# shenwei356/kmcp

Measured on AMD Instinct MI355X. Metric: reads/sec searched (150bp, k=21) vs GTDB-scale index, higher is better.
Workload: dtype u32 bitwise (bit-sliced counters), u64 hashes; 1 GPU; gtdb-scale synthetic: 32 blocks x 14976 cols x 968700 sigs (58.03 GB), 150bp k=21; batch_reads=524288, read_len=150, k=21, num_hashes=1, index_bytes=58029004800, index_bytes_this_rank=58029004800, blocks=32, columns=479232, parallelism=block-shard x1, search_flags=-t 0.55 -c 10 -m 30 -f 0.01 -u 256 -s qcov

## Files before the change

kmcp_amd/csrc/common.hpp:

```cpp
#pragma once
#include <stdint.h>

#include "../../include/kmcp_gpu.h"

namespace kmcpg {

struct BlockDev {
  const uint8_t* rows;
  uint64_t num_sigs;
  uint64_t magic_hi;
  uint32_t stride;
  uint32_t row_bytes;
  uint32_t ncols;
  uint32_t col_base;
  uint32_t seg0, nsegs;
};

struct Seg {
  uint32_t byte_start, byte_end;
  uint32_t col_base;
  uint32_t ncols;
};

struct ExcRun {
  uint64_t pos;
  uint32_t len;
  uint32_t byte;
};

struct Slot {
  uint32_t block;
  uint32_t tile;
};
constexpr uint32_t SLOT_TILE_BITS = 24, SLOT_MAX_TILES = 255;

struct K1Args {
  const uint8_t* seqs;
  const uint64_t* offs;
  const uint8_t* seqs2;
  const uint64_t* offs2;
  uint32_t n_reads;
  int32_t k;
  int32_t min_qlen;
  int32_t scaled;
  uint64_t max_hash;
  int32_t mode;
  uint32_t w_or_s;
  uint64_t* hashes;
  uint64_t* scratch;
  uint64_t* scratch2;
  int32_t* nk_raw;
  int32_t* nk1;
  int32_t* qlen;
  int32_t* seg_cnt;
  uint32_t segs_max;
  int32_t* nk_adj;
  int32_t dedup_threshold;
  int32_t flags;
  uint32_t* seg_list;
  uint32_t* seg_nflag;
  int32_t seg_only_flagged;
  const uint8_t* codes;
  const ExcRun* exc;
  uint32_t n_exc;
  uint8_t* seqs_w;
  uint32_t* seg_exc;
  const uint64_t* src;
};


struct PackedSrc {
  const uint8_t* codes = nullptr;
  const ExcRun* exc = nullptr;
  uint32_t n_exc = 0;
  uint8_t* text = nullptr;
  uint64_t n_bases = 0;
};
constexpr int K1_WIN_CHUNK = 1024;
struct WindowSrc {
  const uint64_t* src = nullptr;
  const uint64_t* soffs = nullptr;
  const uint64_t* wpre = nullptr;
  const uint64_t* cpre = nullptr;
  uint32_t ns = 0;
  uint64_t n_chunks = 0, sb = 0, step = 0, window = 0;
};

struct DedupArgs {
  const uint64_t* offs;
  const uint64_t* offs2;
  uint32_t n_reads;
  int32_t dedup_threshold;
  int32_t min_matched;
  int32_t lo, hi;
  int32_t n_lo, n_hi;
  int32_t pre;
  int32_t pre_done;
  int32_t key_shift;
  uint64_t* hashes;
  uint64_t* scratch;
  const int32_t* nk_raw;
  int32_t* nk_search;
  uint32_t* fallbacks;
};

constexpr int K2_GATHER_SLOTS = 256;

struct K2Args {
  const BlockDev* blocks;
  const Seg* segs;
  const Slot* slots;
  uint32_t nslots;
  uint32_t n_reads;
  const uint64_t* hashes;
  const uint64_t* offs;
  const uint64_t* offs2;
  const int32_t* nk;
  double min_qcov;
  int32_t min_matched;
  int32_t num_hashes;
  int32_t nt_loads;
  int32_t prune;
  int32_t group_rows;
  int32_t prune_every;
  int32_t split_min;
  int32_t slot_major;
  int32_t tail_sectors;
  int32_t tail_min;
  const uint32_t* long_list;
  uint32_t n_long;
  uint32_t split_chk;
  uint32_t split_chunks;
  uint32_t* long_counts;
  uint32_t ncols_total;
  uint64_t unit_base;
  kmcpg_hit* hits;
  uint64_t hit_cap;
  unsigned long long* counter;
  unsigned long long* gathered;
  const uint16_t* cmin_fpr;
  int32_t cmin_fpr_n;
  int32_t k2_flags;
};
static_assert(sizeof(K2Args) == 208, "k2_flags sits in the tail padding: the argument block of every K2 form keeps its layout");

constexpr int K3_WAVE_CAP = 512, K3_WG_CAP = 4096;
struct K3Args {
  const kmcpg_hit* hits;
  const unsigned long long* n_hits;
  uint64_t hit_cap;
  const int32_t* nk;
  uint32_t n_reads;
  uint32_t n_cols;
  const uint64_t* col_size;
  double min_tcov;
  int32_t sort_mode;
  uint32_t* cnt;
  uint64_t* offs;
  uint64_t* sums;
  kmcpg_pair* pairs;
  uint32_t* bad;
};

constexpr int K3_SET_STATS = 4;
struct K3SetArgs {
  uint32_t n_members;
  uint32_t base[16];
  uint32_t* stats;
};

constexpr uint8_t K4_DROP = 0, K4_KEEP = 1, K4_HOST = 2;
constexpr int K4_STATS = 6;
struct K4Args {
  const kmcpg_pair* pairs;
  const uint64_t* offs;
  uint64_t pair_cap;
  const int32_t* nk;
  uint32_t n_reads;
  uint32_t n_cols;
  int32_t final_n;
  const uint32_t* target_class;
  const uint32_t* species_class;
  uint32_t* cnt;
  uint64_t* sums;
  uint8_t* verdict;
  kmcpg_pair* out_pairs;
  uint64_t* out_offs;
  uint64_t out_cap;
  uint32_t* stats;
};

}
```

kmcp_amd/csrc/engine.hpp:

```cpp
#pragma once
#include <stdlib.h>
#include <hip/hip_runtime.h>
#include <stdint.h>

#include <atomic>
#include <condition_variable>
#include <functional>
#include <memory>
#include <mutex>
#include <string>
#include <vector>

#include "../../include/kmcp_gpu.h"
#include "common.hpp"
#include "dbformat.hpp"
#include "k1_plan.hpp"
#include "fpr.hpp"

int kmcpg_fail(int code, const char* fmt, ...);
std::string& kmcpg_err_ref();

#define HIPCHK(expr)                                                                               \
  do {                                                                                             \
    hipError_t e_ = (expr);                                                                        \
    if (e_ != hipSuccess) return kmcpg_fail(KMCPG_EDEVICE, "%s: %s (%s:%d)", #expr, hipGetErrorString(e_), __FILE__, __LINE__); \
  } while (0)

#define KMCPG_NO_FILES_ONLY(db)                                                                                   \
  do {                                                                                                            \
    if ((db)->files_only) return kmcpg_fail(KMCPG_EUNSUPPORTED, "handle of kmcpg_open_files: index inspection only, open the database directory with kmcpg_open to search it"); \
  } while (0)

#define KMCPG_USE_DEVICE(db)                                                                                      \
  do {                                                                                                            \
    if ((db)->opts.device < 0) return kmcpg_fail(KMCPG_EDEVICE, "metadata-only handle (device -1): no GPU work possible"); \
    HIPCHK(hipSetDevice((db)->opts.device));                                                                      \
  } while (0)

namespace kmcpg {

struct BlockMeta {
  std::string path;
  UnikiHeader h;
  uint32_t col_base = 0;
  bool local = false;
  int local_idx = -1;
  uint32_t stride = 0;
  uint8_t* d_rows = nullptr;
  int group = -1;
  uint32_t byte_off = 0;
};

struct Group {
  uint8_t* d_rows = nullptr;
  uint64_t num_sigs = 0;
  uint32_t stride = 0, row_bytes = 0;
  std::vector<int> members;
};

struct SlotClass {
  int lpr = 0;
  std::vector<Slot> slots;
  Slot* d_slots = nullptr;
  std::vector<Slot> bslots;
  Slot* d_bslots = nullptr;
};

template <typename T>
struct DevBuf {
  T* p = nullptr;
  size_t cap = 0;
  int ensure(size_t n) {
    if (n <= cap) return 0;
    if (p) (void)hipFree(p);
    p = nullptr;
    cap = 0;
    size_t want = n + n / 8 + 64;
    if (hipMalloc((void**)&p, want * sizeof(T)) != hipSuccess) return -1;
    cap = want;
    return 0;
  }
  void release() {
    if (p) (void)hipFree(p);
    p = nullptr;
    cap = 0;
  }
};

}

namespace kmcpg {
struct Exchange;
struct FprBoundTable {
  uint64_t key = 0;
  int n = 0;
  uint16_t* d = nullptr;
  uint16_t* h = nullptr;
};
void release_fpr_bounds(kmcpg_db* db);
int plan_passes(kmcpg_db* front, int device, uint64_t* largest_shard_bytes, uint64_t* free_bytes, uint64_t* reserve_bytes = nullptr);
int open_like(const kmcpg_db* src, const kmcpg_opts* opts, kmcpg_db** out);
struct AsyncState;
void async_release(kmcpg_db* db);
int async_in_flight(kmcpg_db* db);
}

struct kmcpg_db {
  kmcpg_opts opts{};
  kmcpg_info info{};
  std::vector<kmcpg::BlockMeta> blocks;
  std::vector<int> local;
  std::vector<kmcpg::BlockDev> h_blockdev;
  kmcpg::BlockDev* d_blockdev = nullptr;
  std::vector<kmcpg::Group> groups;
  std::vector<kmcpg::BlockDev> h_groupdev;
  kmcpg::BlockDev* d_groupdev = nullptr;
  std::vector<kmcpg::Seg> h_segs;
  kmcpg::Seg* d_segs = nullptr;
  std::vector<kmcpg::SlotClass> classes;
  std::vector<uint32_t> col_block;
  struct ColMeta {
    uint64_t size;
    uint64_t gsize;
    uint32_t tidx;
    uint32_t pad;
  };
  std::vector<ColMeta> col_meta;
  std::unique_ptr<kmcpg::QueryFpr> fpr;
  std::mutex mu;
  std::vector<int> ks_desc;
  kmcpg::AsyncState* async = nullptr;
  struct Workspace {
    kmcpg::DevBuf<uint64_t> w_hashes, w_scratch;
    kmcpg::DevBuf<int32_t> w_nk_raw, w_nk1, w_seg_cnt;
    kmcpg::DevBuf<uint32_t> w_long_list, w_long_meta, w_long_counts;
    kmcpg::DevBuf<uint64_t> w_huge_info;
    kmcpg::DevBuf<uint8_t> w_huge_temp;
    kmcpg::DevBuf<uint32_t> w_dedup_fb;
    kmcpg::DevBuf<uint64_t> w_gathered;
    kmcpg::DevBuf<uint64_t> w_win_h, w_win_kept, w_win_cbase;
    kmcpg::DevBuf<uint32_t> w_win_rank, w_win_cnt;
    hipEvent_t ev = nullptr;
    bool ev_valid = false;
    hipEvent_t in_ev = nullptr, k1_ev = nullptr;
    void release() {
      w_hashes.release(); w_scratch.release(); w_nk_raw.release(); w_nk1.release(); w_seg_cnt.release(); w_long_list.release();
      w_long_meta.release(); w_long_counts.release(); w_huge_info.release(); w_huge_temp.release(); w_gathered.release(); w_dedup_fb.release();
      w_win_h.release(); w_win_kept.release(); w_win_cbase.release(); w_win_rank.release(); w_win_cnt.release();
      if (ev) (void)hipEventDestroy(ev);
      if (in_ev) (void)hipEventDestroy(in_ev);
      if (k1_ev) (void)hipEventDestroy(k1_ev);
      ev = in_ev = k1_ev = nullptr;
      ev_valid = false;
    }
  };
  Workspace ws[2];
  uint64_t ws_calls = 0;
  uint64_t k1_codes_direct = 0, k1_codes_expanded = 0;
  int ws_last = 0;
  hipStream_t k1_stream = nullptr;
  hipEvent_t cobs_ev = nullptr;
  bool cobs_ev_valid = false;
  hipEvent_t fin_ev = nullptr;
  bool fin_ev_valid = false;
  bool synthetic = false;
  bool files_only = false;
  float last_density_ms = -1;
  kmcpg_density_launch last_density{};
  std::vector<kmcpg_db*> shards;
  kmcpg::Exchange* exchange = nullptr;
  std::string exchange_why;
  std::string db_dir;
  int paged_passes = 0, paged_device = 0, paged_rank = -1;
  kmcpg_db* paged_resident = nullptr;
  std::mutex paged_mu;
  uint64_t paged_uploads = 0;
  uint64_t paged_reserve = 0;
  int profiling = 0;
  std::vector<kmcpg_k2_launch> k2_log;
  std::vector<kmcpg_k1_launch> k1_log;
  const uint32_t* k1_left = nullptr;
  std::vector<kmcpg_dedup_launch> dedup_log;
  const uint32_t* dedup_fb = nullptr;
  uint64_t* d_col_size = nullptr;
  kmcpg::DevBuf<uint32_t> w_fin_cnt;
  kmcpg::DevBuf<uint64_t> w_fin_sums;
  std::vector<std::string> set_dirs;
  std::vector<uint32_t> set_col_base;
  bool is_set() const { return set_col_base.size() > 1; }
  uint32_t* d_set_stats = nullptr;
  mutable std::atomic<uint64_t> set_host_segments{0}, set_host_mixed{0};
  uint32_t* d_spec_target = nullptr;
  uint32_t* d_spec_species = nullptr;
  std::vector<uint32_t> h_spec_target, h_spec_species;
  bool spec_on() const { return !h_spec_target.empty(); }
  kmcpg::DevBuf<uint32_t> w_spec_cnt;
  kmcpg::DevBuf<uint64_t> w_spec_sums;
  uint64_t* d_spec_stats = nullptr;
  bool spec_ran = false;
  hipEvent_t spec_ev[2] = {};
  bool spec_timed = false;
  std::vector<kmcpg_k4_launch> k4_log;
  std::vector<kmcpg::FprBoundTable> fpr_bounds;
  hipEvent_t ev[16] = {};
  uint64_t ev_calls = 0;
};


namespace kmcpg {

inline int set_refuse_params(const kmcpg_db* db, const kmcpg_params& p) {
  if (!db->is_set()) return 0;
  const char* what = p.try_se ? "try_se" : (p.do_not_sort ? "do_not_sort" : (p.top_n_scores != 0 ? "top_n_scores != 0" : (p.k != 0 ? "params->k != 0" : nullptr)));
  if (!what) return 0;
  return kmcpg_fail(KMCPG_EUNSUPPORTED, "database set (%zu members): %s is not supported — it acts per member in separate searches and would act per query here; "
                    "search the databases one by one and merge the results with kmcp-merge", db->set_col_base.size(), what);
}
inline int set_refuse_entry(const kmcpg_db* db, const char* entry) {
  if (!db->is_set()) return 0;
  return kmcpg_fail(KMCPG_EUNSUPPORTED, "database set (%zu members): %s is not supported on a set handle", db->set_col_base.size(), entry);
}

inline int specific_refuse_params(const kmcpg_db* db, const kmcpg_params& p) {
  if (!db->spec_on()) return 0;
  const char* what = p.try_se ? "try_se" : (p.top_n_scores != 0 ? "top_n_scores != 0" : (p.k == 0 && db->ks_desc.size() > 1 ? "a database with several k-mer sizes searched with params->k == 0" : nullptr));
  if (!what) return 0;
  return kmcpg_fail(KMCPG_EUNSUPPORTED, "species-specific queries (kmcpg_set_specific): %s is not supported — switch the stage off, or filter the results with kmcp-filter", what);
}
inline int specific_refuse_entry(const kmcpg_db* db, const char* entry) {
  if (!db->spec_on()) return 0;
  return kmcpg_fail(KMCPG_EUNSUPPORTED, "species-specific queries (kmcpg_set_specific): %s is not supported while the stage is on", entry);
}

inline kmcpg_params default_params() {
  kmcpg_params p{};
  p.min_qlen = 30;
  p.min_matched = 10;
  p.min_qcov = 0.55;
  p.min_tcov = 0;
  p.max_fpr = 0.01;
  p.dedup_threshold = 256;
  return p;
}

template <class T>
struct NoInitAlloc : std::allocator<T> {
  template <class U>
  struct rebind {
    using other = NoInitAlloc<U>;
  };
  template <class U, class... A>
  void construct(U* q, A&&... a) {
    if constexpr (sizeof...(A) == 0) ::new ((void*)q) U;
    else ::new ((void*)q) U(std::forward<A>(a)...);
  }
};
template <class T>
struct LineAlloc : NoInitAlloc<T> {
  template <class U>
  struct rebind {
    using other = LineAlloc<U>;
  };
  T* allocate(size_t n) {
    void* q = nullptr;
    if (posix_memalign(&q, 64, std::max<size_t>(64, n * sizeof(T))) != 0) throw std::bad_alloc();
    return (T*)q;
  }
  void deallocate(T* q, size_t) { free(q); }
};
typedef std::vector<kmcpg_match, LineAlloc<kmcpg_match>> MatchVec;

struct ResultOwner {
  std::vector<int32_t> qlen, qkmers, ksize;
  std::vector<uint64_t> offs;
  MatchVec matches;
  std::vector<kmcpg_pair, NoInitAlloc<kmcpg_pair>> pairs;
  bool pairs_mode = false;
};
ResultOwner* result_owner_take();
void result_owner_give(ResultOwner* o);
void result_owner_shape(ResultOwner* o, uint32_t n_reads, bool as_pairs);
int finalize_grouped_into(const kmcpg_db* db, const kmcpg_pair* pairs, const uint64_t* read_offs, const int32_t* qkmers, const int32_t* qlen, uint32_t n_reads,
                          const kmcpg_params& p, ResultOwner* o, uint32_t read_base, uint64_t match_base, uint64_t* kept_out, bool trusted = false,
                          int32_t bound_n = 0, const uint8_t* verdicts = nullptr);
int finalize_grouped_trusted(const kmcpg_db* db, const kmcpg_pair* pairs, const uint64_t* read_offs, const int32_t* qkmers, const int32_t* qlen, uint32_t n_reads,
                             const kmcpg_params& p, kmcpg_result* out, int32_t bound_n, bool as_pairs, const uint8_t* verdicts = nullptr);
void specific_filter_result(const kmcpg_db* db, kmcpg_result* out);
inline int k1_mode(const kmcpg_info& I) { return I.syncmer ? 2 : (I.minimizer ? 1 : 0); }
bool whole_genome_batch(const kmcpg_db* db, uint32_t max_read_len, bool paired);
inline bool fpr_bound_enabled() {
  const char* e = getenv("KMCPG_FPR_BOUND");
  return !(e && atoi(e) == 0);
}
constexpr int kFprBoundAlways = 512;
void result_publish(ResultOwner* o, uint32_t n_reads, int k_used, kmcpg_result* out);
struct DeviceBatch {
  const uint8_t* d_seqs = nullptr;
  const uint64_t* d_offs = nullptr;
  const uint8_t* d_seqs2 = nullptr;
  const uint64_t* d_offs2 = nullptr;
// ... 44 lines not shown
```

kmcp_amd/csrc/k2_cobs.hip:

```cpp
#include <hip/hip_runtime.h>

#include <algorithm>
#include <type_traits>

#include "common.hpp"
#include "csa.hpp"
#include "device_utils.hpp"
#include "kernels.hpp"

namespace kmcpg {

typedef uint32_t u32x4 __attribute__((ext_vector_type(4)));
__device__ __forceinline__ uint4 load_row16(const uint8_t* p, int nt) {
  const u32x4* q = reinterpret_cast<const u32x4*>(p);
  const u32x4 v = nt ? __builtin_nontemporal_load(q) : *q;
  return make_uint4(v.x, v.y, v.z, v.w);
}

typedef const u32x4 __attribute__((address_space(1))) * global_row_ptr;
__device__ __forceinline__ uint4 load_row16_global(const uint8_t* p, int nt) {
  global_row_ptr q = (global_row_ptr)(uintptr_t)p;
  const u32x4 v = nt ? __builtin_nontemporal_load(q) : *q;
  return make_uint4(v.x, v.y, v.z, v.w);
}

__device__ __forceinline__ bool group_col(const Seg* __restrict__ segs, const BlockDev* __restrict__ bd, uint32_t byte, uint32_t bit, uint32_t* col) {
  const Seg* s = segs + bd->seg0;
  for (uint32_t i = 0; i < bd->nsegs; i++, s++) {
    if (byte < s->byte_end) {
      const uint32_t c = (byte - s->byte_start) * 8u + (7u - bit);
      *col = s->col_base + c;
      return byte >= s->byte_start && c < s->ncols;
    }
  }
  return false;
}


struct alignas(16) UnitConst {
  uint64_t ns, mh;
  uint64_t koff;
  uint32_t s16;
  int32_t n;
};

template <int NPL>
__device__ __forceinline__ void k2_emit_tile(const K2Args& a, const BlockDev* __restrict__ bd, uint32_t r, uint32_t boff, uint32_t cmin, bool live,
                                             const uint32_t (&pl)[4][NPL], int lane) {
  const bool emit = live && (cmin >> NPL) == 0;
  uint32_t ge[4];
  uint32_t mine = 0;
#pragma unroll
  for (int d = 0; d < 4; d++) {
    uint32_t v = emit ? 0xffffffffu : 0u;
#pragma unroll
    for (int p = 0; p < NPL; p++) v = ((cmin >> p) & 1u) ? (v & pl[d][p]) : (v | pl[d][p]);
    ge[d] = v;
    mine += (uint32_t)__popc(v);
  }
  if (__ballot(mine != 0) == 0) return;
  uint32_t incl = mine;
#pragma unroll
  for (int off = 1; off < 64; off <<= 1) {
    const uint32_t t = __shfl_up(incl, off);
    if (lane >= off) incl += t;
  }
  const uint32_t total = __shfl(incl, 63);
  unsigned long long base_idx = 0;
  if (lane == 63) base_idx = atomicAdd(a.counter, (unsigned long long)total);
  base_idx = __shfl(base_idx, 63);
  unsigned long long idx = base_idx + (incl - mine);
  uint32_t sg_lo = 1, sg_hi = 0, sg_col = 0;
  const Seg* __restrict__ segs = a.segs + bd->seg0;
  const uint32_t nsegs = bd->nsegs;
#pragma unroll
  for (int d = 0; d < 4; d++) {
    uint32_t w = ge[d];
    while (w) {
      const int q = __ffs(w) - 1;
      w &= w - 1;
      uint32_t count = 0;
#pragma unroll
      for (int p = 0; p < NPL; p++) count |= ((pl[d][p] >> q) & 1u) << p;
      const uint32_t byte = boff + (uint32_t)d * 4u + (uint32_t)(q >> 3);
      if (byte < sg_lo || byte >= sg_hi) {
        for (uint32_t i = 0; i < nsegs; i++) {
          const Seg sg = segs[i];
          if (byte < sg.byte_end) {
            sg_lo = sg.byte_start;
            sg_hi = sg.byte_end;
            sg_col = sg.col_base;
            break;
          }
        }
      }
      if (idx < a.hit_cap) {
        kmcpg_hit hit;
        hit.read = r;
        hit.col = sg_col + (byte - sg_lo) * 8u + (7u - (uint32_t)(q & 7));
        hit.count = count;
        if (byte < sg_lo || byte >= sg_hi) hit = kmcpg_hit{0xffffffffu, 0xffffffffu, 0u};
        a.hits[idx] = hit;
      }
      idx++;
    }
  }
}

template <int LPR, int NPL, bool MULTI, bool SPLIT, int GR = 8>
__global__ void __launch_bounds__(256) __attribute__((amdgpu_waves_per_eu((NPL == 16 && !SPLIT && !MULTI && LPR >= 16) ? 3 : 1, (GR == 4 && LPR == 64) ? 4 : 10))) k2_cobs(const K2Args a) {
#define K2_BID blockIdx.x
#include "k2_cobs_body.inc"
#undef K2_BID
}

template <int LPR, int NPL, bool MULTI, bool SPLIT, int GR>
__device__ __forceinline__ void k2_body(const K2Args& a, const unsigned bid) {
#define K2_BID bid
#include "k2_cobs_body.inc"
#undef K2_BID
}


template <int LPRA, int LPRB, int NPL, bool MULTI>
__global__ void __launch_bounds__(256) __attribute__((amdgpu_waves_per_eu((NPL == 16 && !MULTI) ? 3 : 1, 10))) k2_cobs_pair(const K2Args a, const K2Args b, const unsigned nba) {
  if (blockIdx.x < nba) k2_body<LPRA, NPL, MULTI, false, 8>(a, blockIdx.x);
  else k2_body<LPRB, NPL, MULTI, false, 8>(b, blockIdx.x - nba);
}

static void note_k2(K2Log* log, int kind, int lpr, int lprb, int npl, bool multi, int gr, unsigned nb) {
  if (!log) return;
  kmcpg_k2_launch r{};
  r.kind = kind;
  r.lpr = lpr;
  r.lprb = lprb;
  r.npl = npl;
  r.multi = multi ? 1 : 0;
  r.group_rows = gr;
  r.workgroups = nb;
  log->push_back(r);
}

template <int LPR, int NPL, bool MULTI, bool SPLIT, int GR>
static void launch_k2_form(const K2Args& b, unsigned nb, hipStream_t st, K2Log* log) {
  hipLaunchKernelGGL((k2_cobs<LPR, NPL, MULTI, SPLIT, GR>), dim3(nb), dim3(256), 0, st, b);
  note_k2(log, SPLIT ? 1 : 0, LPR, 0, NPL, MULTI, GR, nb);
}

template <int LPRA, int LPRB, int NPL, bool MULTI>
static void launch_k2_pair_form(const K2Args& a, const K2Args& b, unsigned nba, unsigned nbb, hipStream_t st, K2Log* log) {
  hipLaunchKernelGGL((k2_cobs_pair<LPRA, LPRB, NPL, MULTI>), dim3(nba + nbb), dim3(256), 0, st, a, b, nba);
  note_k2(log, 2, LPRA, LPRB, NPL, MULTI, 8, nba + nbb);
}

template <int LPR, int NPL, bool SPLIT, int GR>
static int launch_k2_pieces(const K2Launch& l, const K2Args& a, hipStream_t st, K2Log* log) {
  K2Args b = a;
  for (uint64_t i = 0, n = k2_n_pieces(l); i < n; i++) {
    const K2Piece pc = k2_piece(l, i);
    b.unit_base = pc.unit_base;
    if (l.multi)
      launch_k2_form<LPR, NPL, true, SPLIT, GR>(b, pc.workgroups, st, log);
    else
      launch_k2_form<LPR, NPL, false, SPLIT, GR>(b, pc.workgroups, st, log);
  }
  return 0;
}

template <int LPR>
static int launch_k2_plain_l(const K2Launch& l, const K2Args& a, hipStream_t st, K2Log* log) {
  const bool four = l.gr == 4;
  if (!four && l.gr != 8) return -1;
  switch (l.npl) {
    case 8: return four ? launch_k2_pieces<LPR, 8, false, 4>(l, a, st, log) : launch_k2_pieces<LPR, 8, false, 8>(l, a, st, log);
    case 10: return four ? launch_k2_pieces<LPR, 10, false, 4>(l, a, st, log) : launch_k2_pieces<LPR, 10, false, 8>(l, a, st, log);
    case 16: return four ? -1 : launch_k2_pieces<LPR, 16, false, 8>(l, a, st, log);
    case 24: return four ? -1 : launch_k2_pieces<LPR, 24, false, 8>(l, a, st, log);
    default: return -1;
  }
}

static int launch_k2_plain(const K2Launch& l, const K2Args& a, hipStream_t st, K2Log* log) {
  switch (l.lpr) {
    case 4: return launch_k2_plain_l<4>(l, a, st, log);
    case 8: return launch_k2_plain_l<8>(l, a, st, log);
    case 16: return launch_k2_plain_l<16>(l, a, st, log);
    case 32: return launch_k2_plain_l<32>(l, a, st, log);
    case 64: return launch_k2_plain_l<64>(l, a, st, log);
    default: return -1;
  }
}

template <int LPRB>
static int launch_k2_pair_l(const K2Launch& l, const K2Args& a, const K2Args& b, hipStream_t st, K2Log* log) {
  if (l.multi)
    launch_k2_pair_form<64, LPRB, 16, true>(a, b, l.nba, l.nbb, st, log);
  else
    launch_k2_pair_form<64, LPRB, 16, false>(a, b, l.nba, l.nbb, st, log);
  return 0;
}

int launch_k2_pair(const K2Launch& l, const K2Args& a, const K2Args& b, hipStream_t st, K2Log* log) {
  if (l.kind != K2Kind::Pair || l.lpr != 64 || l.npl != 16 || l.gr != 8) return -1;
  switch (l.lprb) {
    case 32: return launch_k2_pair_l<32>(l, a, b, st, log);
    case 16: return launch_k2_pair_l<16>(l, a, b, st, log);
    case 8: return launch_k2_pair_l<8>(l, a, b, st, log);
    case 4: return launch_k2_pair_l<4>(l, a, b, st, log);
    default: return -1;
  }
}

int launch_k2(const K2Launch& l, const K2Args& a, hipStream_t st, K2Log* log) {
  if (l.kind == K2Kind::Plain) return launch_k2_plain(l, a, st, log);
  if (l.kind != K2Kind::Split || l.npl != 16 || l.gr != 8) return -1;
  switch (l.lpr) {
    case 4: return launch_k2_pieces<4, 16, true, 8>(l, a, st, log);
    case 8: return launch_k2_pieces<8, 16, true, 8>(l, a, st, log);
    case 16: return launch_k2_pieces<16, 16, true, 8>(l, a, st, log);
    case 32: return launch_k2_pieces<32, 16, true, 8>(l, a, st, log);
    case 64: return launch_k2_pieces<64, 16, true, 8>(l, a, st, log);
    default: return -1;
  }
}

__global__ void k_list_long(const int32_t* __restrict__ nk, uint32_t n_reads, int32_t split_min, uint32_t* __restrict__ list, uint32_t* __restrict__ meta) {
  const uint32_t r = blockIdx.x * blockDim.x + threadIdx.x;
  if (r < n_reads && nk[r] > split_min) {
    list[atomicAdd(&meta[0], 1u)] = r;
    atomicMax(&meta[1], (uint32_t)nk[r]);
  }
}

void launch_list_long(const int32_t* nk, uint32_t n_reads, int32_t split_min, uint32_t* list, uint32_t* meta, hipStream_t st) {
  if (n_reads == 0) return;
  hipLaunchKernelGGL(k_list_long, dim3((n_reads + 255) / 256), dim3(256), 0, st, nk, n_reads, split_min, list, meta);
}

__global__ void k_max_nk(const int32_t* __restrict__ nk, uint32_t n_reads, unsigned long long* __restrict__ out) {
  int m = 0;
  for (uint32_t r = blockIdx.x * blockDim.x + threadIdx.x; r < n_reads; r += gridDim.x * blockDim.x) m = max(m, nk[r]);
#pragma unroll
  for (int off = 32; off >= 1; off >>= 1) m = max(m, __shfl_xor(m, off));
  if ((threadIdx.x & 63) == 0 && m > 0) atomicMax(out, (unsigned long long)m);
}

void launch_max_nk(const int32_t* nk, uint32_t n_reads, unsigned long long* out, hipStream_t st) {
  if (n_reads == 0) return;
  const unsigned blocks = std::min<unsigned>(1024, (n_reads + 255) / 256);
  hipLaunchKernelGGL(k_max_nk, dim3(blocks), dim3(256), 0, st, nk, n_reads, out);
}

__global__ void k_threshold_long(const K2Args a) {
  const uint64_t total = (uint64_t)a.n_long * a.ncols_total;
  const int lane = threadIdx.x & 63;
  const uint64_t step = (uint64_t)gridDim.x * blockDim.x;
  for (uint64_t i0 = (uint64_t)blockIdx.x * blockDim.x + (threadIdx.x & ~63u); i0 < total; i0 += step) {
    const uint64_t i = i0 + (uint64_t)lane;
    uint32_t c = 0, r = 0, col = 0;
    bool pass = false;
    if (i < total && (c = a.long_counts[i]) != 0) {
      const uint32_t li = (uint32_t)(i / a.ncols_total);
      col = (uint32_t)(i % a.ncols_total);
      r = a.long_list[li];
      const int n = a.nk[r];
      uint32_t cmin = count_threshold(n, a.min_qcov, a.min_matched);
      if (a.cmin_fpr && n <= a.cmin_fpr_n) cmin = max(cmin, (uint32_t)a.cmin_fpr[n]);
      pass = c >= cmin;
    }
    const uint64_t m = __ballot(pass);
    if (m == 0) continue;
    const int leader = __ffsll((unsigned long long)m) - 1;
    unsigned long long base = 0;
    if (lane == leader) base = atomicAdd(a.counter, (unsigned long long)__popcll(m));
    base = __shfl(base, leader);
    if (pass) {
      const unsigned long long idx = base + (unsigned long long)__popcll(m & ((1ULL << lane) - 1ULL));
      if (idx < a.hit_cap) {
        kmcpg_hit hit;
        hit.read = r;
        hit.col = col;
        hit.count = c;
        a.hits[idx] = hit;
      }
    }
  }
}

void launch_threshold_long(const K2Args& a, hipStream_t st) {
  const uint64_t total = (uint64_t)a.n_long * a.ncols_total;
  if (total == 0) return;
  unsigned blocks = (unsigned)((total + 255) / 256 > 65536 ? 65536 : (total + 255) / 256);
  hipLaunchKernelGGL(k_threshold_long, dim3(blocks), dim3(256), 0, st, a);
}

}
```

kmcp_amd/csrc/query.cpp:

```cpp
#include <hip/hip_runtime.h>
#include <math.h>
#include <stdarg.h>
#include <stdio.h>
#include <stdlib.h>
#include <errno.h>
#include <fcntl.h>
#include <string.h>
#include <unistd.h>

#include <algorithm>
#include <atomic>
#include <memory>
#include <mutex>
#include <string>
#include <thread>
#include <unordered_map>
#include <vector>

#include "common.hpp"
#include "dbformat.hpp"
#include "engine.hpp"
#include "fpr.hpp"
#include "kernels.hpp"

// ... 383 lines not shown
  if (int rc = window_spec_args(spec)) return rc;
  if (n_windows && !n_slices) return kmcpg_fail(KMCPG_EINVAL, "windows without a staged slice");
  if ((uint64_t)max_window_len > spec->window || window_bases > (uint64_t)n_windows * max_window_len || n_chunks > staged_bases)
    return kmcpg_fail(KMCPG_EINVAL, "the piece's sizes contradict each other");
  WindowPiece w;
  w.d_text = d_text;
  w.d_soffs = d_soffs;
  w.d_wpre = d_wpre;
  w.d_vpre = d_vpre;
  w.d_cpre = d_cpre;
  w.ns = n_slices;
  w.sb = staged_bases;
  w.n_chunks = n_chunks;
  w.n_win = n_windows;
  w.wmax = max_window_len;
  w.bases = window_bases;
  w.step = spec->step;
  w.window = spec->window;
  w.d_src = d_src;
  w.d_offs = d_koff;
  hipStream_t st = (hipStream_t)stream;
  const std::function<int()> desc = [&]() -> int { return describe_windows(w, st); };
  return kmers_device(db, w.batch(), params, d_hashes, hashes_cap, nullptr, d_nk, nullptr, stream, d_qlen, &desc);
}

extern "C" int kmcpg_k1_codes_batches(kmcpg_db* db, uint64_t* direct, uint64_t* expanded) {
  if (!db) return kmcpg_fail(KMCPG_EINVAL, "null argument");
  std::lock_guard<std::mutex> g(db->mu);
  if (direct) *direct = db->k1_codes_direct;
  if (expanded) *expanded = db->k1_codes_expanded;
  return 0;
}

extern "C" int kmcpg_query_device(kmcpg_db* db, const uint8_t* d_seqs, const uint64_t* d_offs, const uint8_t* d_seqs2, const uint64_t* d_offs2,
                                  uint32_t n_reads, uint64_t total_bases, uint32_t max_read_len, const kmcpg_params* params, kmcpg_hit* d_hits,
                                  uint64_t hit_cap, uint64_t* d_counters, int32_t* d_qkmers, int32_t* d_qlen, void* stream) {
  return kmcpg::query_device_after(db, DeviceBatch{d_seqs, d_offs, d_seqs2, d_offs2, n_reads, total_bases, max_read_len}, params,
                                   QueryOut{d_hits, hit_cap, d_counters, d_qkmers, d_qlen}, stream, nullptr, nullptr);
}

int kmcpg::query_device_after(kmcpg_db* db, const DeviceBatch& b, const kmcpg_params* params, const QueryOut& out, void* stream,
                              const std::function<int()>* prologue, int32_t* bound_n) {
  if (!db || !b.d_seqs || !b.d_offs || !out.d_counters || !out.d_qkmers || !out.d_qlen || (!out.d_hits && out.hit_cap)) return kmcpg_fail(KMCPG_EINVAL, "null argument");
  if ((b.d_seqs2 == nullptr) != (b.d_offs2 == nullptr)) return kmcpg_fail(KMCPG_EINVAL, "seqs2 and offs2 must be given together");
  KMCPG_NO_FILES_ONLY(db);
  std::lock_guard<std::mutex> g(db->mu);
  KMCPG_USE_DEVICE(db);
  if (prologue)
    if (int rcp = (*prologue)()) return rcp;
  const kmcpg_params p = params ? *params : default_params();
  if (int rcs = set_refuse_params(db, p)) return rcs;
  if (p.min_matched < 1) return kmcpg_fail(KMCPG_EINVAL, "min_matched must be >= 1");
  if (p.k > 0 && std::find(db->ks_desc.begin(), db->ks_desc.end(), p.k) == db->ks_desc.end())
    return kmcpg_fail(KMCPG_EINVAL, "k=%d is not a k-mer size of this database", p.k);
  const int k_used = p.k > 0 ? p.k : db->info.k;
  hipStream_t st = (hipStream_t)stream;
  static const bool test_hooks = getenv("KMCPG_TEST_HOOKS") && atoi(getenv("KMCPG_TEST_HOOKS")) == 1;
  if (test_hooks)
    if (const char* e = getenv("KMCPG_TEST_MAX_BASES"))
      if (b.total_bases > (uint64_t)atoll(e)) return kmcpg_fail(KMCPG_ENOMEM, "hipMalloc failed (KMCPG_TEST_MAX_BASES)");
  const int slot = pick_slot(db, b.total_bases, whole_genome_batch(db, b.max_read_len, b.d_seqs2 != nullptr));
  db->ws_calls++;
  db->ws_last = slot;
  db->k2_log.clear();
  K2Log* const k2_log = db->profiling >= 1 ? &db->k2_log : nullptr;
  kmcpg_db::Workspace& W = db->ws[slot];
  static const bool k1_own = getenv("KMCPG_K1_STREAM") && atoi(getenv("KMCPG_K1_STREAM")) == 1;
  hipStream_t kst = st;
  if (k1_own) {
    if (!db->k1_stream) {
      int lo = 0, hi = 0;
      if (hipDeviceGetStreamPriorityRange(&lo, &hi) != hipSuccess) lo = hi = 0;
      HIPCHK(hipStreamCreateWithPriority(&db->k1_stream, hipStreamNonBlocking, hi));
    }
    if (!W.in_ev) HIPCHK(hipEventCreateWithFlags(&W.in_ev, hipEventDisableTiming));
    if (!W.k1_ev) HIPCHK(hipEventCreateWithFlags(&W.k1_ev, hipEventDisableTiming));
    kst = db->k1_stream;
    HIPCHK(hipEventRecord(W.in_ev, st));
    HIPCHK(hipStreamWaitEvent(kst, W.in_ev, 0));
  }
  if (int rc0 = ws_begin(W, kst)) return rc0;
  WsGuard wsg{W, st, kst};
  if (W.w_hashes.ensure(b.total_bases + 1) || W.w_nk_raw.ensure(b.n_reads + 1) || W.w_nk1.ensure(b.n_reads + 1)) return kmcpg_fail(KMCPG_ENOMEM, "hipMalloc failed");
  uint64_t ub = b.max_read_len >= (uint32_t)k_used ? (uint64_t)(b.max_read_len - k_used + 1) : 0;
  if (b.d_seqs2) ub *= 2;
  const bool window_sketch = db->info.syncmer || db->info.minimizer;
  if ((ub > (uint64_t)p.dedup_threshold || window_sketch) && W.w_scratch.ensure(2 * b.total_bases + 2)) return kmcpg_fail(KMCPG_ENOMEM, "hipMalloc failed");
  uint64_t maxn = 0;
  hipEvent_t* pev = db->ev + 4 * (db->ev_calls % 4);
  if (db->profiling) {
    for (auto& ev : db->ev)
      if (!ev) HIPCHK(hipEventCreate(&ev));
    HIPCHK(hipEventRecord(pev[0], kst));
  }
  int rc = run_kmers(db, W, b, p, KmerOut{W.w_hashes.p, W.w_scratch.p, b.total_bases + 1, W.w_nk_raw.p, W.w_nk1.p, out.d_qkmers, out.d_qlen}, kst, &maxn);
  if (rc) return rc;
  HIPCHK(hipMemsetAsync(out.d_counters, 0, 2 * sizeof(uint64_t), kst));
  launch_max_nk(out.d_qkmers, b.n_reads, (unsigned long long*)out.d_counters + 1, kst);
  if (db->profiling) HIPCHK(hipEventRecord(pev[3], kst));
  if (k1_own) {
    HIPCHK(hipEventRecord(W.k1_ev, kst));
    HIPCHK(hipStreamWaitEvent(st, W.k1_ev, 0));
  }
  static const int debug_rowsort = getenv("KMCPG_DEBUG_ROWSORT") ? atoi(getenv("KMCPG_DEBUG_ROWSORT")) : 0;
  if (debug_rowsort && !b.d_offs2 && !db->h_groupdev.empty())
    launch_debug_rowsort(W.w_hashes.p, b.d_offs, out.d_qkmers, b.n_reads, db->h_groupdev[0].num_sigs, db->h_groupdev[0].magic_hi, debug_rowsort, st);
  K2Shape s;
  s.n_reads = b.n_reads;
  s.max_n = maxn;
  s.num_hashes = db->info.num_hashes;
  s.matrix_bytes_local = db->info.matrix_bytes_local;
  s.n_cols = db->info.n_cols;
  if (db->classes.size() > (size_t)K2_MAX_CLASSES) return kmcpg_fail(KMCPG_EINVAL, "more lane classes than lane forms");
  for (const auto& c : db->classes) s.classes[s.n_classes++] = K2Class{c.lpr, (uint32_t)c.slots.size(), c.d_bslots ? (uint32_t)c.bslots.size() : 0u};
  s.knobs = k2_knobs();
  uint32_t long_meta[2] = {0, 0};
  const bool ask = k2_ask_long(s);
  if (ask) {
    if (W.w_long_list.ensure(b.n_reads + 1) || W.w_long_meta.ensure(2)) return kmcpg_fail(KMCPG_ENOMEM, "hipMalloc failed");
    HIPCHK(hipMemsetAsync(W.w_long_meta.p, 0, 2 * sizeof(uint32_t), st));
    launch_list_long(out.d_qkmers, b.n_reads, s.knobs.split_min, W.w_long_list.p, W.w_long_meta.p, st);
    HIPCHK(hipMemcpyAsync(long_meta, W.w_long_meta.p, sizeof long_meta, hipMemcpyDeviceToHost, st));
    HIPCHK(hipStreamSynchronize(st));
  }
  const K2Plan plan = k2_plan(s, ask, long_meta[0], long_meta[1]);
  if (!plan.npl) return kmcpg_fail(KMCPG_EUNSUPPORTED, "queries with more than 16777214 k-mers need KMCPG_SPLIT_MIN > 0");
  K2Args a{};
  a.blocks = db->d_groupdev;
  a.segs = db->d_segs;
  a.n_reads = b.n_reads;
  a.hashes = W.w_hashes.p;
  a.offs = b.d_offs;
  a.offs2 = b.d_offs2;
  a.nk = out.d_qkmers;
  a.min_qcov = p.min_qcov;
  a.min_matched = p.min_matched;
  a.num_hashes = db->info.num_hashes;
  a.nt_loads = s.knobs.nt_loads;
  a.prune = s.knobs.prune;
  a.group_rows = plan.group_rows;
  a.prune_every = plan.prune_every;
  a.split_min = plan.split_min;
  a.slot_major = s.knobs.slot_major;
  a.tail_sectors = s.knobs.tail_sectors;
  a.tail_min = s.knobs.tail_min;
  a.hits = out.d_hits;
  a.hit_cap = out.hit_cap;
  a.counter = (unsigned long long*)out.d_counters;
  if (db->profiling >= 2) {
    if (W.w_gathered.ensure((size_t)K2_GATHER_SLOTS * 16)) return kmcpg_fail(KMCPG_ENOMEM, "hipMalloc failed");
    HIPCHK(hipMemsetAsync(W.w_gathered.p, 0, (size_t)K2_GATHER_SLOTS * 16 * sizeof(uint64_t), st));
    a.gathered = (unsigned long long*)W.w_gathered.p;
  }
  if (int rcb = fpr_bound(db, p.max_fpr, plan.max_short, st, &a.cmin_fpr, &a.cmin_fpr_n)) return rcb;
  if (bound_n) *bound_n = a.cmin_fpr ? a.cmin_fpr_n : 0;
  static const bool cobs_chain = !(getenv("KMCPG_COBS_CHAIN") && atoi(getenv("KMCPG_COBS_CHAIN")) == 0);
  if (int rcc = chain_begin(&db->cobs_ev, cobs_chain && db->cobs_ev_valid, st)) return rcc;
  if (db->profiling) HIPCHK(hipEventRecord(pev[1], st));
  auto with_slots = [&](K2Args x, int cls, const K2Launch& l) {
    const SlotClass& c = db->classes[(size_t)cls];
    x.slots = l.block_units ? c.d_bslots : c.d_slots;
    x.nslots = l.block_units ? (uint32_t)c.bslots.size() : (uint32_t)c.slots.size();
    x.k2_flags = l.k2_flags;
    return x;
  };
  const char* const no_kernel = "batch too large for one launch: split it";
  for (int i = 0; i < plan.n_launches; i++) {
    const K2Launch& l = plan.launches[i];
    if (l.kind == K2Kind::Split) continue;
    const int rcl = l.kind == K2Kind::Pair ? launch_k2_pair(l, with_slots(a, l.cls, l), with_slots(a, l.cls_b, l), st, k2_log) : launch_k2(l, with_slots(a, l.cls, l), st, k2_log);
    if (rcl != 0) return kmcpg_fail(KMCPG_EINVAL, no_kernel);
  }
  if (plan.n_long) {
    a.ncols_total = (uint32_t)db->info.n_cols;
    a.split_chk = plan.split_chk;
    a.split_chunks = plan.split_chunks;
    if (W.w_long_counts.ensure((size_t)std::min<uint32_t>(plan.group, plan.n_long) * a.ncols_total)) return kmcpg_fail(KMCPG_ENOMEM, "hipMalloc failed");
    a.long_counts = W.w_long_counts.p;
    for (uint32_t g0 = 0; g0 < plan.n_long; g0 += plan.group) {
      a.long_list = W.w_long_list.p + g0;
      a.n_long = std::min<uint32_t>(plan.group, plan.n_long - g0);
      HIPCHK(hipMemsetAsync(a.long_counts, 0, (size_t)a.n_long * a.ncols_total * sizeof(uint32_t), st));
      for (int i = 0; i < plan.n_launches; i++) {
        const K2Launch& l = plan.launches[i];
        if (l.kind == K2Kind::Split && launch_k2(k2_split_launch(plan, s, l, a.n_long), with_slots(a, l.cls, l), st, k2_log) != 0)
          return kmcpg_fail(KMCPG_EINVAL, no_kernel);
      }
      launch_threshold_long(a, st);
    }
  }
  HIPCHK(hipEventRecord(db->cobs_ev, st));
  db->cobs_ev_valid = true;
  if (db->profiling) {
    HIPCHK(hipEventRecord(pev[2], st));
    db->ev_calls++;
  }
  if (int rc1 = wsg.finish()) return rc1;
  HIPCHK(hipGetLastError());
  return 0;
}

extern "C" int kmcpg_group_device(kmcpg_db* db, const kmcpg_hit* d_hits, const uint64_t* d_n_hits, uint64_t hit_cap, const int32_t* d_qkmers, uint32_t n_reads,
                                  const kmcpg_params* params, kmcpg_pair* d_pairs, uint64_t* d_read_offs, void* stream) {
  if (!db || !d_n_hits || !d_read_offs || (n_reads && !d_qkmers) || (hit_cap && (!d_hits || !d_pairs))) return kmcpg_fail(KMCPG_EINVAL, "null argument");
  if (db->opts.device < 0 || !db->d_col_size) return kmcpg_fail(KMCPG_EDEVICE, "metadata-only handle (device -1): no GPU work possible");
  std::lock_guard<std::mutex> g(db->mu);
  KMCPG_USE_DEVICE(db);
  const kmcpg_params p = params ? *params : default_params();
  if (int rcs = set_refuse_params(db, p)) return rcs;
  hipStream_t st = (hipStream_t)stream;
  if (int rc0 = chain_begin(&db->fin_ev, db->fin_ev_valid, st)) return rc0;
  struct FinGuard {
    kmcpg_db* db;
    hipStream_t st;
    ~FinGuard() {
      if (db->fin_ev && hipEventRecord(db->fin_ev, st) == hipSuccess) db->fin_ev_valid = true;
    }
  } fing{db, st};
  if (db->w_fin_cnt.ensure((size_t)n_reads + 2) || db->w_fin_sums.ensure((size_t)k3_scan_tiles_for(n_reads + 1) + 1)) return kmcpg_fail(KMCPG_ENOMEM, "hipMalloc failed");
  HIPCHK(hipMemsetAsync(db->w_fin_cnt.p, 0, ((size_t)n_reads + 2) * sizeof(uint32_t), st));
  K3Args a{};
  a.hits = d_hits;
  a.n_hits = (const unsigned long long*)d_n_hits;
  a.hit_cap = hit_cap;
  a.nk = d_qkmers;
  a.n_reads = n_reads;
  a.n_cols = (uint32_t)db->col_meta.size();
  a.col_size = db->d_col_size;
  a.min_tcov = p.min_tcov;
  a.sort_mode = p.do_not_sort ? 3 : (p.sort_by == 1 ? 1 : (p.sort_by == 2 ? 2 : 0));
  a.cnt = db->w_fin_cnt.p;
  a.bad = db->w_fin_cnt.p + n_reads + 1;
  a.offs = d_read_offs;
  a.sums = db->w_fin_sums.p;
  a.pairs = d_pairs;
  if (n_reads == 0) HIPCHK(hipMemsetAsync(d_read_offs, 0, 2 * sizeof(uint64_t), st));
  else {
    K3SetArgs sa{};
    if (db->is_set()) {
      sa.n_members = (uint32_t)db->set_col_base.size();
      for (uint32_t i = 0; i < sa.n_members; i++) sa.base[i] = db->set_col_base[i];
      sa.stats = db->d_set_stats;
      HIPCHK(hipMemsetAsync(db->d_set_stats, 0, K3_SET_STATS * sizeof(uint32_t), st));
      db->set_host_segments.store(0);
      db->set_host_mixed.store(0);
    }
    launch_k3(a, 0, st, db->is_set() ? &sa : nullptr);
    HIPCHK(hipMemsetAsync(d_read_offs + n_reads + 1, 0, sizeof(uint64_t), st));
    HIPCHK(hipMemcpyAsync(d_read_offs + n_reads + 1, a.bad, sizeof(uint32_t), hipMemcpyDeviceToDevice, st));
  }
  HIPCHK(hipGetLastError());
  return 0;
}

extern "C" int kmcpg_set_profiling(kmcpg_db* db, int enable) {
  if (!db) return kmcpg_fail(KMCPG_EINVAL, "null argument");
  std::lock_guard<std::mutex> g(db->mu);
  db->profiling = enable < 0 ? 0 : (enable > 2 ? 2 : enable);
  db->ev_calls = 0;
  return 0;
}

static int read_gather_slots(kmcpg_db* db, int word, uint64_t unit, uint64_t* bytes) {
  if (!db || !bytes) return kmcpg_fail(KMCPG_EINVAL, "null argument");
  std::lock_guard<std::mutex> g(db->mu);
  kmcpg_db::Workspace& W = db->ws[db->ws_last];
  if (db->profiling < 2 || !W.w_gathered.p || db->ev_calls == 0) return kmcpg_fail(KMCPG_EINVAL, "no kmcpg_query_device call at profiling level 2 yet");
  KMCPG_USE_DEVICE(db);
  hipEvent_t* pev = db->ev + 4 * ((db->ev_calls - 1) % 4);
  HIPCHK(hipEventSynchronize(pev[2]));
  std::vector<uint64_t> slots((size_t)K2_GATHER_SLOTS * 16);
  HIPCHK(hipMemcpy(slots.data(), W.w_gathered.p, slots.size() * sizeof(uint64_t), hipMemcpyDeviceToHost));
  uint64_t n = 0;
  for (int i = 0; i < K2_GATHER_SLOTS; i++) n += slots[(size_t)i * 16 + (size_t)word];
  *bytes = n * unit;
  return 0;
}

extern "C" int kmcpg_last_gathered_bytes(kmcpg_db* db, uint64_t* bytes) { return read_gather_slots(db, 0, 16, bytes); }
extern "C" int kmcpg_last_hash_bytes(kmcpg_db* db, uint64_t* bytes) { return read_gather_slots(db, 1, 8, bytes); }
extern "C" int kmcpg_last_tail_waves(kmcpg_db* db, uint64_t* waves) { return read_gather_slots(db, 2, 1, waves); }

extern "C" int kmcpg_last_k2_launches(kmcpg_db* db, kmcpg_k2_launch* out, uint32_t cap, uint32_t* n) {
  static_assert(sizeof(kmcpg_k2_launch) == 32, "eight 4-byte words");
  if (!db || !n || (cap && !out)) return kmcpg_fail(KMCPG_EINVAL, "null argument");
  std::lock_guard<std::mutex> g(db->mu);
  if (db->profiling < 1) return kmcpg_fail(KMCPG_EINVAL, "no kmcpg_query_device call at profiling level >= 1 yet");
  const size_t m = std::min<size_t>(cap, db->k2_log.size());
  if (m) memcpy(out, db->k2_log.data(), m * sizeof(kmcpg_k2_launch));
  *n = (uint32_t)db->k2_log.size();
  return 0;
}

extern "C" int kmcpg_last_k1_launches(kmcpg_db* db, kmcpg_k1_launch* out, uint32_t cap, uint32_t* n) {
  static_assert(sizeof(kmcpg_k1_launch) == 32, "eight 4-byte words");
  if (!db || !n || (cap && !out)) return kmcpg_fail(KMCPG_EINVAL, "null argument");
  std::lock_guard<std::mutex> g(db->mu);
  const size_t have = db->profiling >= 1 ? db->k1_log.size() : 0;
  const size_t m = std::min<size_t>(cap, have);
  if (m) memcpy(out, db->k1_log.data(), m * sizeof(kmcpg_k1_launch));
  *n = (uint32_t)have;
  return 0;
}

extern "C" int kmcpg_last_dedup_launches(kmcpg_db* db, kmcpg_dedup_launch* out, uint32_t cap, uint32_t* n) {
  static_assert(sizeof(kmcpg_dedup_launch) == 32, "eight 4-byte words");
// ... 83 lines not shown
```

Baseline: 1.095 million reads/s.

## Add persistent K2 COBS kernel with atomic work queue for single-tile plain launches

Adds a persistent-workgroup form of the K2 bit-sliced counter search. A grid sized to resident occupancy claims runs of (read, slot) units from a global atomic counter, so the non-persistent grid is replaced by dynamic load balancing. Slot metadata is cached across consecutive units that share a slot. It applies only to plain launches with 64 lanes per row, group_rows 4 and nonzero k2_flags, and is on by default. The cost is an extra queue memset and atomics per claim, plus a different occupancy profile (waves_per_eu capped at 4).

```diff
diff --git a/kmcp_amd/csrc/common.hpp b/kmcp_amd/csrc/common.hpp
--- a/kmcp_amd/csrc/common.hpp
+++ b/kmcp_amd/csrc/common.hpp
@@ -1,4 +1,5 @@
 #pragma once
+#include <stddef.h>
 #include <stdint.h>
 
 #include "../../include/kmcp_gpu.h"
@@ -141,8 +142,11 @@
   const uint16_t* cmin_fpr;
   int32_t cmin_fpr_n;
   int32_t k2_flags;
+  unsigned long long* unit_queue;
+  uint32_t persist_wgs;
 };
-static_assert(sizeof(K2Args) == 208, "k2_flags sits in the tail padding: the argument block of every K2 form keeps its layout");
+constexpr int K2_QUEUE_PITCH = 16;
+static_assert(sizeof(K2Args) == 224 && offsetof(K2Args, unit_queue) == 208, "new fields go behind k2_flags: what the other K2 forms read keeps its place in the argument block");
 
 constexpr int K3_WAVE_CAP = 512, K3_WG_CAP = 4096;
 struct K3Args {
diff --git a/kmcp_amd/csrc/engine.hpp b/kmcp_amd/csrc/engine.hpp
--- a/kmcp_amd/csrc/engine.hpp
+++ b/kmcp_amd/csrc/engine.hpp
@@ -138,6 +138,7 @@
     kmcpg::DevBuf<uint8_t> w_huge_temp;
     kmcpg::DevBuf<uint32_t> w_dedup_fb;
     kmcpg::DevBuf<uint64_t> w_gathered;
+    kmcpg::DevBuf<uint64_t> w_k2_queue;
     kmcpg::DevBuf<uint64_t> w_win_h, w_win_kept, w_win_cbase;
     kmcpg::DevBuf<uint32_t> w_win_rank, w_win_cnt;
     hipEvent_t ev = nullptr;
@@ -146,6 +147,7 @@
     void release() {
       w_hashes.release(); w_scratch.release(); w_nk_raw.release(); w_nk1.release(); w_seg_cnt.release(); w_long_list.release();
       w_long_meta.release(); w_long_counts.release(); w_huge_info.release(); w_huge_temp.release(); w_gathered.release(); w_dedup_fb.release();
+      w_k2_queue.release();
       w_win_h.release(); w_win_kept.release(); w_win_cbase.release(); w_win_rank.release(); w_win_cnt.release();
       if (ev) (void)hipEventDestroy(ev);
       if (in_ev) (void)hipEventDestroy(in_ev);
diff --git a/kmcp_amd/csrc/k2_claim.hpp b/kmcp_amd/csrc/k2_claim.hpp
--- /dev/null
+++ b/kmcp_amd/csrc/k2_claim.hpp
@@ -0,0 +1,36 @@
+#pragma once
+#include <stdint.h>
+
+#include "k2_plan.hpp"
+
+#if defined(__HIPCC__)
+#define K2_CLAIM_HD __host__ __device__ inline
+#else
+#define K2_CLAIM_HD inline
+#endif
+
+namespace kmcpg {
+
+constexpr uint32_t K2_CLAIM_RUN = 8;
+
+struct K2Run {
+  uint64_t first, last;
+};
+
+K2_CLAIM_HD K2Run k2_claim_run(uint64_t ticket, uint64_t unit_base, uint64_t units, uint32_t run) {
+  const uint64_t lo = ticket < units ? ticket : units;
+  const uint64_t hi = units - lo < run ? units : lo + run;
+  return K2Run{unit_base + lo, unit_base + hi};
+}
+
+K2_CLAIM_HD uint64_t k2_piece_units(uint64_t total_units, uint64_t unit_base, uint64_t piece_workgroups) {
+  const uint64_t left = total_units > unit_base ? total_units - unit_base : 0;
+  return left < piece_workgroups * 4 ? left : piece_workgroups * 4;
+}
+
+K2_CLAIM_HD unsigned k2_persist_grid(unsigned piece_workgroups, unsigned resident, uint32_t asked) {
+  const unsigned nb = asked ? asked : (piece_workgroups < resident ? piece_workgroups : resident);
+  return nb < 1 ? 1 : (nb > (unsigned)K2_MAX_BLOCKS ? (unsigned)K2_MAX_BLOCKS : nb);
+}
+
+}
diff --git a/kmcp_amd/csrc/k2_cobs.hip b/kmcp_amd/csrc/k2_cobs.hip
--- a/kmcp_amd/csrc/k2_cobs.hip
+++ b/kmcp_amd/csrc/k2_cobs.hip
@@ -6,6 +6,7 @@
 #include "common.hpp"
 #include "csa.hpp"
 #include "device_utils.hpp"
+#include "k2_claim.hpp"
 #include "kernels.hpp"
 
 namespace kmcpg {
@@ -121,6 +122,175 @@
 #undef K2_BID
 }
 
+struct K2UnitQueue {
+  static constexpr uint64_t NONE = ~0ull;
+  unsigned long long* counter;
+  uint64_t unit_base, units;
+  int lane;
+  uint64_t cur = 0, end = 0;
+  __device__ __forceinline__ uint64_t take() {
+    if (cur == end) {
+      unsigned long long tk = 0;
+      if (lane == 0) tk = atomicAdd(counter, (unsigned long long)K2_CLAIM_RUN);
+      const uint64_t t = (uint64_t)(uint32_t)__builtin_amdgcn_readfirstlane((int)(uint32_t)tk) |
+                         ((uint64_t)(uint32_t)__builtin_amdgcn_readfirstlane((int)(uint32_t)(tk >> 32)) << 32);
+      const K2Run r = k2_claim_run(t, unit_base, units, K2_CLAIM_RUN);
+      cur = r.first;
+      end = r.last;
+      if (cur == end) return NONE;
+    }
+    return cur++;
+  }
+};
+
+template <int NPL>
+__global__ void __launch_bounds__(256) __attribute__((amdgpu_waves_per_eu(1, 4))) k2_cobs_persist(const K2Args a, const unsigned piece_workgroups, unsigned long long* __restrict__ queue) {
+  constexpr int NMAX = NPL == 8 ? 256 : 1024;
+  __shared__ uint32_t s_all[4][NMAX + 4];
+  const int lane = threadIdx.x & 63, wave = threadIdx.x >> 6;
+  const bool exact = (a.k2_flags & K2F_EXACT_STOP) != 0;
+  const int sec0 = lane & ~7;
+  auto uni = [](uint32_t v) __attribute__((always_inline)) -> uint32_t { return (uint32_t)__builtin_amdgcn_readfirstlane((int)v); };
+  auto uni64 = [&](uint64_t v) __attribute__((always_inline)) -> uint64_t { return (uint64_t)uni((uint32_t)v) | ((uint64_t)uni((uint32_t)(v >> 32)) << 32); };
+
+  K2UnitQueue q{queue, a.unit_base, k2_piece_units((uint64_t)a.n_reads * a.nslots, a.unit_base, piece_workgroups), lane};
+  uint32_t cur_sidx = 0xffffffffu, tb = 0, s16 = 0;
+  const BlockDev* __restrict__ bd = nullptr;
+  const uint8_t* __restrict__ tbase = nullptr;
+  uint64_t ns = 0, mh = 0;
+  bool lv0 = false;
+  uint32_t g_rows = 0;
+  uint64_t g_hashes = 0;
+  for (;;) {
+    const uint64_t u = q.take();
+    if (u == K2UnitQueue::NONE) break;
+    const uint32_t sidx = (uint32_t)(a.slot_major ? u / a.n_reads : u % a.nslots);
+    const uint32_t r0 = (uint32_t)(a.slot_major ? u % a.n_reads : u / a.nslots);
+    if (sidx != cur_sidx) {
+      cur_sidx = sidx;
+      const Slot slot = a.slots[sidx];
+      bd = a.blocks + uni(slot.block);
+      const uint32_t stride = uni(bd->stride);
+      ns = uni64(bd->num_sigs);
+      mh = uni64(bd->magic_hi);
+      s16 = stride >> 4;
+      tb = (uni(slot.tile) * 64u + (uint32_t)lane) * 16u;
+      tbase = (const uint8_t*)uni64((uint64_t)(uintptr_t)bd->rows) + tb;
+      lv0 = tb < stride;
+    }
+    int n0 = (int)uni((uint32_t)a.nk[r0]);
+    if ((a.split_min > 0 && n0 > a.split_min) || n0 > NMAX) n0 = 0;
+    if (n0 == 0) continue;
+    {
+      const uint64_t koff = uni64(a.offs[r0] + (a.offs2 ? a.offs2[r0] : 0));
+      for (int c0 = 0; c0 < n0; c0 += 256) {
+        uint64_t hv[4];
+#pragma unroll
+        for (int it = 0; it < 4; it++) hv[it] = c0 + 64 * it + lane < n0 ? a.hashes[koff + (uint64_t)(c0 + 64 * it + lane)] : 0;
+#pragma unroll
+        for (int it = 0; it < 4; it++)
+          if (c0 + 64 * it + lane < n0) s_all[wave][c0 + 64 * it + lane] = (uint32_t)fastmod_u64(hv[it], ns, mh) * s16;
+      }
+      wave_lds_fence();
+    }
+    uint32_t cmin0 = count_threshold(n0, a.min_qcov, a.min_matched);
+    if (a.cmin_fpr && n0 <= a.cmin_fpr_n) cmin0 = max(cmin0, (uint32_t)a.cmin_fpr[n0]);
+    cmin0 = uni(cmin0);
+    const int cm0 = (int)min(cmin0, 1u << NPL);
+    bool lv = lv0;
+    uint32_t cp[4][NPL];
+#pragma unroll
+    for (int d = 0; d < 4; d++)
+#pragma unroll
+    for (int p = 0; p < NPL; p++) cp[d][p] = 0;
+    const int nn = n0, cm = cm0;
+    auto at_least = [&](int t_) __attribute__((always_inline)) -> bool {
+      uint32_t w[NPL];
+#pragma unroll
+      for (int p = 0; p < NPL; p++) w[p] = (((uint32_t)t_ >> p) & 1u) - 1u;
+      uint32_t any = 0;
+#pragma unroll
+      for (int d = 0; d < 4; d++) {
+        uint32_t ge = 0xffffffffu;
+#pragma unroll
+        for (int p = 0; p < NPL; p++) ge = MAJ3(ge, cp[d][p], w[p]);
+        any |= ge;
+      }
+      return t_ <= 0 || (((uint32_t)t_ >> NPL) == 0 && any != 0);
+    };
+    auto in_sector = [&](bool b) __attribute__((always_inline)) -> bool { return ((__ballot(b) >> sec0) & 0xffull) != 0; };
+    int done = 0;
+    int sdone = 0;
+    int credit = 0;
+    bool try_far = true;
+    for (;;) {
+      int L, rem;
+      if (exact) {
+        rem = nn - done;
+        const int need = cm - rem;
+        credit = max(credit, 1 - need);
+        const int want_rows = min(4, rem);
+        bool ask_ = lv && credit < want_rows;
+        if (__ballot(ask_) != 0) {
+          if (try_far) {
+            const bool far = in_sector(lv && at_least(need + 15));
+            credit = ask_ && far ? 16 : credit;
+            ask_ = ask_ && !far;
+            try_far = __ballot(ask_) == 0;
+          }
+          if (__ballot(ask_) != 0) {
+            const bool top = in_sector(lv && at_least(need + 3));
+            credit = ask_ && top ? 4 : credit;
+            ask_ = ask_ && !top;
+            if (__ballot(ask_) != 0) {
+              const bool t1 = in_sector(lv && at_least(need + 1));
+              const bool t2 = in_sector(lv && at_least(t1 ? need + 2 : need));
+              const int fine = t1 ? (t2 ? 3 : 2) : (t2 ? 1 : 0);
+              credit = ask_ ? fine : credit;
+              lv = lv && !(ask_ && fine == 0);
+            }
+          }
+        }
+        L = lv ? min(credit, want_rows) : 0;
+        credit -= L;
+      } else {
+        rem = nn - sdone;
+        L = in_sector(lv && at_least(cm - rem)) ? 4 : 0;
+        sdone += min(4, rem);
+        lv = lv && L > 0;
+        L = lv ? min(L, rem) : 0;
+      }
+      if (__ballot(L > 0) == 0) break;
+      uint32_t ri[4];
+      uint4 x[4];
+#pragma unroll
+      for (int i = 0; i < 4; i++) ri[i] = s_all[wave][done + i];
+#pragma unroll
+      for (int i = 0; i < 4; i++) {
+        x[i] = make_uint4(0, 0, 0, 0);
+        if (i < L) x[i] = load_row16_global(tbase + ((uint64_t)ri[i] << 4), a.nt_loads);
+      }
+      csa4<NPL>(cp[0], x[0].x, x[1].x, x[2].x, x[3].x);
+      csa4<NPL>(cp[1], x[0].y, x[1].y, x[2].y, x[3].y);
+      csa4<NPL>(cp[2], x[0].z, x[1].z, x[2].z, x[3].z);
+      csa4<NPL>(cp[3], x[0].w, x[1].w, x[2].w, x[3].w);
+      done += L;
+      g_rows += (uint32_t)L;
+    }
+    g_hashes += (uint64_t)nn;
+    k2_emit_tile<NPL>(a, bd, r0, tb, cmin0, lv, cp, lane);
+  }
+  if (a.gathered) {
+    unsigned long long rows = g_rows;
+#pragma unroll
+    for (int off = 32; off >= 1; off >>= 1) rows += __shfl_xor(rows, off);
+    if (lane == 0) {
+      atomicAdd(a.gathered + (size_t)(blockIdx.x % K2_GATHER_SLOTS) * 16, rows);
+      atomicAdd(a.gathered + (size_t)(blockIdx.x % K2_GATHER_SLOTS) * 16 + 1, (unsigned long long)g_hashes);
+    }
+  }
+}
+
 
 template <int LPRA, int LPRB, int NPL, bool MULTI>
 __global__ void __launch_bounds__(256) __attribute__((amdgpu_waves_per_eu((NPL == 16 && !MULTI) ? 3 : 1, 10))) k2_cobs_pair(const K2Args a, const K2Args b, const unsigned nba) {
@@ -153,12 +323,30 @@
   note_k2(log, 2, LPRA, LPRB, NPL, MULTI, 8, nba + nbb);
 }
 
+template <int NPL>
+static int launch_k2_persist_form(const K2Args& b, const K2Piece& pc, uint64_t piece, hipStream_t st, K2Log* log) {
+  int dev = 0, cus = 0, per_cu = 0;
+  if (hipGetDevice(&dev) != hipSuccess || hipDeviceGetAttribute(&cus, hipDeviceAttributeMultiprocessorCount, dev) != hipSuccess ||
+      hipOccupancyMaxActiveBlocksPerMultiprocessor(&per_cu, k2_cobs_persist<NPL>, 256, 0) != hipSuccess || cus <= 0 || per_cu <= 0)
+    return -1;
+  const unsigned nb = k2_persist_grid(pc.workgroups, (unsigned)cus * (unsigned)per_cu, b.persist_wgs);
+  hipLaunchKernelGGL((k2_cobs_persist<NPL>), dim3(nb), dim3(256), 0, st, b, pc.workgroups, b.unit_queue + piece * K2_QUEUE_PITCH);
+  note_k2(log, 0, 64, 0, NPL, false, 4, pc.workgroups);
+  return 0;
+}
+
 template <int LPR, int NPL, bool SPLIT, int GR>
 static int launch_k2_pieces(const K2Launch& l, const K2Args& a, hipStream_t st, K2Log* log) {
   K2Args b = a;
   for (uint64_t i = 0, n = k2_n_pieces(l); i < n; i++) {
     const K2Piece pc = k2_piece(l, i);
     b.unit_base = pc.unit_base;
+    if constexpr (LPR == 64 && NPL <= 10 && !SPLIT && GR == 4) {
+      if (!l.multi && b.unit_queue && b.k2_flags != 0 && !(b.k2_flags & K2F_BLOCK_UNITS)) {
+        if (launch_k2_persist_form<NPL>(b, pc, i, st, log) != 0) return -1;
+        continue;
+      }
+    }
     if (l.multi)
       launch_k2_form<LPR, NPL, true, SPLIT, GR>(b, pc.workgroups, st, log);
     else
diff --git a/kmcp_amd/csrc/query.cpp b/kmcp_amd/csrc/query.cpp
--- a/kmcp_amd/csrc/query.cpp
+++ b/kmcp_amd/csrc/query.cpp
@@ -559,6 +559,19 @@
     HIPCHK(hipMemsetAsync(W.w_gathered.p, 0, (size_t)K2_GATHER_SLOTS * 16 * sizeof(uint64_t), st));
     a.gathered = (unsigned long long*)W.w_gathered.p;
   }
+  if (!(getenv("KMCPG_K2_PERSIST") && atoi(getenv("KMCPG_K2_PERSIST")) == 0)) {
+    uint64_t pieces = 0;
+    for (int i = 0; i < plan.n_launches; i++) {
+      const K2Launch& l = plan.launches[i];
+      if (l.kind == K2Kind::Plain && l.lpr == 64 && l.gr == 4 && l.k2_flags != 0 && !l.block_units) pieces = std::max(pieces, k2_n_pieces(l));
+    }
+    if (pieces) {
+      if (W.w_k2_queue.ensure((size_t)pieces * K2_QUEUE_PITCH)) return kmcpg_fail(KMCPG_ENOMEM, "hipMalloc failed");
+      HIPCHK(hipMemsetAsync(W.w_k2_queue.p, 0, (size_t)pieces * K2_QUEUE_PITCH * sizeof(uint64_t), st));
+      a.unit_queue = (unsigned long long*)W.w_k2_queue.p;
+      if (const char* e = getenv("KMCPG_K2_PERSIST_WGS")) a.persist_wgs = (uint32_t)std::max(0, atoi(e));
+    }
+  }
   if (int rcb = fpr_bound(db, p.max_fpr, plan.max_short, st, &a.cmin_fpr, &a.cmin_fpr_n)) return rcb;
   if (bound_n) *bound_n = a.cmin_fpr ? a.cmin_fpr_n : 0;
   static const bool cobs_chain = !(getenv("KMCPG_COBS_CHAIN") && atoi(getenv("KMCPG_COBS_CHAIN")) == 0);
```

Result: faster. 1.155 million reads/s (median of 6 runs) (+5.4%).
